# GloryyrolG/MHEntropy

Hardware: AMD Instinct MI355X
Metric: hypotheses/sec (BxK) fwd+loss, 256x256 (higher is better)
Workload: dtype bf16; 1 GPU; c2: MHEnt.get_loss forward+loss, resnet50 encoder (train-mode BN), 12-coupling RealNVP h=512, MANO joints, B=256/GPU, K=64, 256x256; images_per_gpu=256, hypotheses_per_image=64, global_batch=256, launch=hip-graph replay, base_noise=drawn on the device inside the step (Philox4x32-10, mhe_randn_f32), timing=one window of 452 steps, bracketed by barrier + synchronize, ranks=1, rccl_ranks=0

## Files before the change

### mhentropy_amd/csrc/conv_stream.hip

```cpp
#include "conv_shared.h"

namespace mhe { namespace conv {

constexpr int ST_PIX = 64;

template <int KT, int ST_BN, bool BNLOAD, bool DG = false>
__global__ __launch_bounds__(256, (ST_BN * KT + 2 * ST_PIX * KT) * 128 + ST_PIX * ST_BN * 2 <= 80 * 1024 ? 2 : 1)
void conv1x1_stream_kernel(const Params p, int nchunks, int ntiles_n) {
    using T = u16;
    constexpr int NTH = 256, CPR = ST_BN * 2 / 16;
    constexpr int NTW = ST_BN / 64, NJ = ST_PIX * CPR / NTH;
    constexpr int SWM = CPR < 16 ? CPR - 1 : 15;
    __shared__ uint4 Wl[ST_BN * 8 * KT];
    __shared__ uint4 Al[2][ST_PIX * 8 * KT];
    __shared__ uint4 Ol[ST_PIX * CPR > NTH * 4 ? ST_PIX * CPR : NTH * 4];
    const int tid = threadIdx.x, wave = tid >> 6, lane = tid & 63, q = lane >> 4, l15 = lane & 15;
    const int nt_id = blockIdx.x % ntiles_n, wg = blockIdx.x / ntiles_n, nwg = gridDim.x / ntiles_n;
    const int n0 = nt_id * ST_BN;
    const int s = tid & 7, rbase = tid >> 3;
    const T *xg = reinterpret_cast<const T *>(p.x);
    const T *wg_ = reinterpret_cast<const T *>(p.w);
    T *yg = reinterpret_cast<T *>(p.y);

#pragma unroll
    for (int kt = 0; kt < KT; ++kt)
#pragma unroll
        for (int j = 0; j < ST_BN / 32; ++j) {
            const int r = rbase + 32 * j, n = n0 + r;
            const uint4 v = n < p.Cout ? *reinterpret_cast<const uint4 *>(wg_ + (size_t)n * p.Kpad + kt * 64 + s * 8) : make_uint4(0, 0, 0, 0);
            Wl[kt * ST_BN * 8 + swz(r, s)] = v;
        }
    float sc[KT][8], sh[KT][8];
    if constexpr (BNLOAD) {
#pragma unroll
        for (int kt = 0; kt < KT; ++kt)
#pragma unroll
            for (int i = 0; i < 8; ++i) { sc[kt][i] = p.in_scale[kt * 64 + s * 8 + i]; sh[kt][i] = p.in_shift[kt * 64 + s * 8 + i]; }
    }
    uint4 ra[KT][2];
    auto load_chunk = [&](int c) {
#pragma unroll
        for (int kt = 0; kt < KT; ++kt)
#pragma unroll
            for (int j = 0; j < 2; ++j) {
                const long m = (long)c * ST_PIX + rbase + 32 * j;
                ra[kt][j] = (c < nchunks && m < p.M) ? *reinterpret_cast<const uint4 *>(xg + (size_t)m * p.Cin + kt * 64 + s * 8) : make_uint4(0, 0, 0, 0);
            }
    };
    auto store_chunk = [&](int buf, int c) {
#pragma unroll
        for (int kt = 0; kt < KT; ++kt)
#pragma unroll
            for (int j = 0; j < 2; ++j) {
                uint4 v = ra[kt][j];
                if constexpr (BNLOAD) {
                    const long m = (long)c * ST_PIX + rbase + 32 * j;
                    if (m < p.M) {
                        float f[8];
                        Chunk<T>::unpack(v, f);
#pragma unroll
                        for (int i = 0; i < 8; ++i) {
                            f[i] = fmaf(f[i], sc[kt][i], sh[kt][i]);
                            if (p.relu_in) f[i] = fmaxf(f[i], 0.f);
                        }
                        v = Chunk<T>::pack(f);
                    }
                }
                Al[buf][kt * ST_PIX * 8 + swz(rbase + 32 * j, s)] = v;
            }
    };
    const bool st_on = !DG && p.stats != nullptr;
    float ss1[8], ss2[8];
#pragma unroll
    for (int i = 0; i < 8; ++i) ss1[i] = ss2[i] = 0.f;
    const int ccol = n0 + (tid % CPR) * 8;
    const T *mk = reinterpret_cast<const T *>(p.mask), *rg = reinterpret_cast<const T *>(p.residual);
    const T *y0g = reinterpret_cast<const T *>(p.bn_y[0]), *y1g = reinterpret_cast<const T *>(p.bn_y[1]);
    const unsigned char *mkb = DG ? p.mask_bits : nullptr;
    const bool y0sum = DG && y0g != nullptr && y0g == mk, y1sum = DG && y1g != nullptr && y1g == mk;
    float bs1[DG ? 2 : 1][8], bs2[DG ? 2 : 1][8], bmu[DG ? 2 : 1][8], biv[DG ? 2 : 1][8];
    if constexpr (DG) {
#pragma unroll
        for (int u = 0; u < 2; ++u)
#pragma unroll
            for (int i = 0; i < 8; ++i) {
                const bool ok = p.bn_y[u] != nullptr && ccol + i < p.Cout;
                bs1[u][i] = bs2[u][i] = 0.f;
                bmu[u][i] = ok ? p.bn_mi[u][ccol + i] : 0.f;
                biv[u][i] = ok ? p.bn_mi[u][p.Cout + ccol + i] : 0.f;
            }
    }

    uint4 gm[DG ? 4 : 1], rr[DG ? 4 : 1], ya[DG ? 4 : 1], yb[DG ? 4 : 1];
    unsigned gmb[DG ? 4 : 1];
    size_t off[DG ? 4 : 1];
    bool okr[DG ? 4 : 1];
    auto dg_load = [&](int j0, int c) __attribute__((always_inline)) {
        if constexpr (DG) {
#pragma unroll
            for (int g = 0; g < 4; ++g) {
                const int id = tid + NTH * (j0 + g), row = id / CPR;
                const long m = (long)c * ST_PIX + row;
                okr[g] = m < p.M && ccol < p.Cout;
                const long mc = okr[g] ? m : 0;
                off[g] = (size_t)mc * p.Cout + ccol;
                if (mkb) gmb[g] = mkb[(size_t)mc * (p.Cout / 8) + (ccol >> 3)];
                else gm[g] = *reinterpret_cast<const uint4 *>(mk + off[g]);
                rr[g] = make_uint4(0u, 0u, 0u, 0u);
                if (rg) {
                    if (p.res_s2) {
                        const long hr = res_half_row(p, mc);
                        if (hr >= 0) rr[g] = *reinterpret_cast<const uint4 *>(rg + (size_t)hr * p.Cout + ccol);
                    } else rr[g] = *reinterpret_cast<const uint4 *>(rg + off[g]);
                }
                if (y0g && !y0sum) ya[g] = *reinterpret_cast<const uint4 *>(y0g + off[g]);
                if (y1g && !y1sum) yb[g] = *reinterpret_cast<const uint4 *>(y1g + off[g]);
            }
        }
    };
    load_chunk(wg);
    int it = 0;
    for (int c = wg; c < nchunks; c += nwg, ++it) {
        const int buf = it & 1;
        store_chunk(buf, c);
        load_chunk(c + nwg);
        if constexpr (ST_BN <= 128) dg_load(0, c);
        __syncthreads();
        v4f acc[NTW][4];
#pragma unroll
        for (int a = 0; a < NTW; ++a)
#pragma unroll
            for (int b = 0; b < 4; ++b) acc[a][b] = v4f{0.f, 0.f, 0.f, 0.f};
#pragma unroll
        for (int kt = 0; kt < KT; ++kt)
#pragma unroll
            for (int kk = 0; kk < 2; ++kk) {
                uint4 fa[4], fb[NTW];
#pragma unroll
                for (int mt = 0; mt < 4; ++mt) fa[mt] = Al[buf][kt * ST_PIX * 8 + swz(mt * 16 + l15, kk * 4 + q)];
#pragma unroll
                for (int nt = 0; nt < NTW; ++nt) fb[nt] = Wl[kt * ST_BN * 8 + swz(wave * (ST_BN / 4) + nt * 16 + l15, kk * 4 + q)];
#pragma unroll
                for (int nt = 0; nt < NTW; ++nt)
#pragma unroll
                    for (int mt = 0; mt < 4; ++mt)
                        acc[nt][mt] = __builtin_amdgcn_mfma_f32_16x16x32_bf16(
                            __builtin_bit_cast(__attribute__((ext_vector_type(8))) __bf16, fb[nt]),
                            __builtin_bit_cast(__attribute__((ext_vector_type(8))) __bf16, fa[mt]), acc[nt][mt], 0, 0, 0);
            }
        {
            unsigned char *ot = reinterpret_cast<unsigned char *>(Ol);
#pragma unroll
            for (int nt = 0; nt < NTW; ++nt)
#pragma unroll
                for (int mt = 0; mt < 4; ++mt) {
                    const int row = mt * 16 + l15, boff = (wave * (ST_BN / 4) + nt * 16 + 4 * q) * 2;
                    const int chunk = (boff >> 4) ^ (row & SWM);
                    const v4f v = acc[nt][mt];
                    uint2 o;
                    o.x = (unsigned)f32_to_bf16(v[0]) | ((unsigned)f32_to_bf16(v[1]) << 16);
                    o.y = (unsigned)f32_to_bf16(v[2]) | ((unsigned)f32_to_bf16(v[3]) << 16);
                    *reinterpret_cast<uint2 *>(ot + ((size_t)row * CPR + chunk) * 16 + (boff & 15)) = o;
                }
        }
        __syncthreads();
        {
            const unsigned char *ot = reinterpret_cast<const unsigned char *>(Ol);
            if constexpr (DG) {
#pragma unroll 1
                for (int j0 = 0; j0 < NJ; j0 += 4) {
                    if (j0 || ST_BN > 128) dg_load(j0, c);
                    uint4 raw[4];
#pragma unroll
                    for (int g = 0; g < 4; ++g) {
                        const int id = tid + NTH * (j0 + g), row = id / CPR, cc = id % CPR;
                        raw[g] = *reinterpret_cast<const uint4 *>(ot + ((size_t)row * CPR + (cc ^ (row & SWM))) * 16);
                    }
#pragma unroll
                    for (int g = 0; g < 4; ++g) {
                        if (!okr[g]) continue;
                        float v[8], t[8];
                        Chunk<T>::unpack(raw[g], v);
                        if (rg) {
                            Chunk<T>::unpack(rr[g], t);
#pragma unroll
                            for (int i = 0; i < 8; ++i) v[i] += t[i];
                        }
                        if (mkb) {
#pragma unroll
                            for (int i = 0; i < 8; ++i) v[i] = ((gmb[g] >> i) & 1u) ? v[i] : 0.f;
                        } else {
                            Chunk<T>::unpack(gm[g], t);
#pragma unroll
                            for (int i = 0; i < 8; ++i) v[i] = t[i] > 0.f ? v[i] : 0.f;
                        }
                        if (y0sum) {
#pragma unroll
                            for (int i = 0; i < 8; ++i) bs1[0][i] += v[i];
                        } else if (y0g) {
                            Chunk<T>::unpack(ya[g], t);
#pragma unroll
                            for (int i = 0; i < 8; ++i) { bs1[0][i] += v[i]; bs2[0][i] = fmaf(v[i], (t[i] - bmu[0][i]) * biv[0][i], bs2[0][i]); }
                        }
                        if (y1sum) {
#pragma unroll
                            for (int i = 0; i < 8; ++i) bs1[1][i] += v[i];
                        } else if (y1g) {
                            Chunk<T>::unpack(yb[g], t);
#pragma unroll
                            for (int i = 0; i < 8; ++i) { bs1[1][i] += v[i]; bs2[1][i] = fmaf(v[i], (t[i] - bmu[1][i]) * biv[1][i], bs2[1][i]); }
                        }
                        *reinterpret_cast<uint4 *>(yg + off[g]) = Chunk<T>::pack(v);
                    }
                }
                continue;
            }
            uint4 raw[NJ];
#pragma unroll
            for (int j = 0; j < NJ; ++j) {
                const int id = tid + NTH * j, row = id / CPR, cc = id % CPR;
                raw[j] = *reinterpret_cast<const uint4 *>(ot + ((size_t)row * CPR + (cc ^ (row & SWM))) * 16);
            }
#pragma unroll
            for (int j = 0; j < NJ; ++j) {
                const int id = tid + NTH * j, row = id / CPR, cc = id % CPR;
                const long m = (long)c * ST_PIX + row;
                const int n = n0 + cc * 8;
                if (m < p.M && n < p.Cout) {
                    if (st_on) {
                        float f[8];
                        Chunk<T>::unpack(raw[j], f);
#pragma unroll
                        for (int i = 0; i < 8; ++i) { ss1[i] += f[i]; ss2[i] = fmaf(f[i], f[i], ss2[i]); }
                    }
                    if (yg) *reinterpret_cast<uint4 *>(yg + (size_t)m * p.Cout + n) = raw[j];
                }
            }
        }
    }
    if constexpr (DG) {
        float *red = reinterpret_cast<float *>(Ol);
#pragma unroll
        for (int u = 0; u < 2; ++u) {
            if (!p.bn_y[u]) continue;
            __syncthreads();
#pragma unroll
            for (int i = 0; i < 8; ++i) { red[tid * 16 + i] = bs1[u][i]; red[tid * 16 + 8 + i] = bs2[u][i]; }
            __syncthreads();
            const int cch = tid / 8, e = tid % 8, n = n0 + tid;
            float a = 0.f, b = 0.f;
            if (tid < ST_BN)
                for (int k = 0; k < NTH / CPR; ++k) { a += red[(cch + CPR * k) * 16 + e]; b += red[(cch + CPR * k) * 16 + 8 + e]; }
            if (tid < ST_BN && n < p.Cout) {
                fx::add(p.bn_stats[u], wg % NSH, 0, p.Cout, n, a);
                fx::add(p.bn_stats[u], wg % NSH, 1, p.Cout, n, b);
            }
        }
    }
    if (st_on) {
        float *red = reinterpret_cast<float *>(Ol);
        __syncthreads();
#pragma unroll
        for (int i = 0; i < 8; ++i) { red[tid * 16 + i] = ss1[i]; red[tid * 16 + 8 + i] = ss2[i]; }
        __syncthreads();
        const int cch = tid / 8, e = tid % 8, n = n0 + tid;
        float a = 0.f, b = 0.f;
        if (tid < ST_BN)
            for (int k = 0; k < NTH / CPR; ++k) { a += red[(cch + CPR * k) * 16 + e]; b += red[(cch + CPR * k) * 16 + 8 + e]; }
        if (tid < ST_BN && n < p.Cout) {
            const int shard = wg % NSH;
            fx::add(p.stats, shard, 0, p.Cout, n, a);
            fx::add(p.stats, shard, 1, p.Cout, n, b);
        }
    }
}

__device__ __forceinline__ int swz3(int row, int slot) { return row * 8 + (slot ^ (((row >> 1) & 3) << 1)); }

template <bool BNLOAD, bool DG>
__global__ __launch_bounds__(512) void conv3x3_c64_stream_kernel(const Params p) {
    using T = u16;
    constexpr int NTH = 512, NT2 = 256, CPR = 8, WPX = 64, RROW = (WPX + 2) * 8;
    __shared__ uint4 Wl[9 * 64 * 8];
    __shared__ uint4 Rl[6][RROW];
    __shared__ uint4 Ol[2][1024];
    const int tid = threadIdx.x, wave = tid >> 6, lane = tid & 63, q = lane >> 4, l15 = lane & 15;
    const bool mult = wave < 4;
    const int t2 = tid & (NT2 - 1);
    const int s = t2 & 7, pbase = t2 >> 3;
    const int wrow = (wave >> 1) & 1, wpx = (wave & 1) * 32;
    const T *xg = reinterpret_cast<const T *>(p.x);
    const T *wg_ = reinterpret_cast<const T *>(p.w);
    T *yg = reinterpret_cast<T *>(p.y);
    const int H = p.H;
    const int npair = (H + 1) / 2 + 1;
    const int nimg = (p.B - (int)blockIdx.x + (int)gridDim.x - 1) / (int)gridDim.x;
    const int NT = nimg * npair;
    for (int i = tid; i < 9 * 64 * 8; i += NTH) {
        const int sl = i & 7, co = (i >> 3) & 63, tap = i >> 9;
        Wl[tap * 512 + swz3(co, sl)] = *reinterpret_cast<const uint4 *>(wg_ + (size_t)co * p.Kpad + tap * 64 + sl * 8);
    }
    if (tid < 6 * 16) {
        const int b = tid >> 4, sl = tid & 7, px = (tid & 8) ? WPX + 1 : 0;
        Rl[b][swz3(px, sl)] = make_uint4(0, 0, 0, 0);
    }
    const bool st_on = !DG && p.stats != nullptr;
    float ss1[8], ss2[8];
#pragma unroll
    for (int i = 0; i < 8; ++i) ss1[i] = ss2[i] = 0.f;
    const int ccol = (t2 % CPR) * 8;
    float bs1[DG ? 2 : 1][8], bs2[DG ? 2 : 1][8];
#pragma unroll
    for (int u = 0; u < (DG ? 2 : 1); ++u)
#pragma unroll
        for (int i = 0; i < 8; ++i) bs1[u][i] = bs2[u][i] = 0.f;

    if (mult) {
        int ck = 0, sp = 2, sc_ = 0;
        for (int t = 0; t <= NT; ++t) {
            __syncthreads();
            if (t < NT && ck >= 1) {
                v4f acc[4][2];
#pragma unroll
                for (int a = 0; a < 4; ++a) { acc[a][0] = v4f{0.f, 0.f, 0.f, 0.f}; acc[a][1] = v4f{0.f, 0.f, 0.f, 0.f}; }
                uint4 fa[2][2], fb[2][4];
                auto frag = [&](int i, int bi) __attribute__((always_inline)) {
                    const int kh = i / 6, kw = (i / 2) % 3, kk = i & 1;
                    const int d = wrow + kh;
                    const uint4 *row = Rl[(d < 2 ? sp : sc_) * 2 + (d & 1)];
#pragma unroll
                    for (int mt = 0; mt < 2; ++mt) fa[bi][mt] = row[swz3(wpx + mt * 16 + l15 + kw, kk * 4 + q)];
#pragma unroll
                    for (int nt = 0; nt < 4; ++nt) fb[bi][nt] = Wl[(kh * 3 + kw) * 512 + swz3(nt * 16 + l15, kk * 4 + q)];
                };
                frag(0, 0);
#pragma unroll
                for (int i = 0; i < 18; ++i) {
                    if (i + 1 < 18) frag(i + 1, (i + 1) & 1);
                    __builtin_amdgcn_sched_barrier(0);
#pragma unroll
                    for (int nt = 0; nt < 4; ++nt)
#pragma unroll
                        for (int mt = 0; mt < 2; ++mt)
                            acc[nt][mt] = __builtin_amdgcn_mfma_f32_16x16x32_bf16(
                                __builtin_bit_cast(__attribute__((ext_vector_type(8))) __bf16, fb[i & 1][nt]),
                                __builtin_bit_cast(__attribute__((ext_vector_type(8))) __bf16, fa[i & 1][mt]), acc[nt][mt], 0, 0, 0);
                    __builtin_amdgcn_sched_barrier(0);
                }
                unsigned char *ot = reinterpret_cast<unsigned char *>(Ol[t & 1]);
#pragma unroll
                for (int nt = 0; nt < 4; ++nt)
#pragma unroll
                    for (int mt = 0; mt < 2; ++mt) {
                        const int row = wrow * WPX + wpx + mt * 16 + l15, boff = (nt * 16 + 4 * q) * 2;
                        const int chunk = (boff >> 4) ^ (row & 7);
                        const v4f v = acc[nt][mt];
                        uint2 o;
                        o.x = (unsigned)f32_to_bf16(v[0]) | ((unsigned)f32_to_bf16(v[1]) << 16);
                        o.y = (unsigned)f32_to_bf16(v[2]) | ((unsigned)f32_to_bf16(v[3]) << 16);
                        *reinterpret_cast<uint2 *>(ot + ((size_t)row * CPR + chunk) * 16 + (boff & 15)) = o;
                    }
            }
            sp = sc_;
            sc_ = sc_ == 2 ? 0 : sc_ + 1;
            if (++ck == npair) ck = 0;
        }
    } else {
        float sc[8], sh[8];
        if constexpr (BNLOAD) {
#pragma unroll
            for (int i = 0; i < 8; ++i) { sc[i] = p.in_scale[s * 8 + i]; sh[i] = p.in_shift[s * 8 + i]; }
        }
        const T *mk = reinterpret_cast<const T *>(p.mask), *rg = reinterpret_cast<const T *>(p.residual);
        const T *y0g = reinterpret_cast<const T *>(p.bn_y[0]), *y1g = reinterpret_cast<const T *>(p.bn_y[1]);
        float bmu[DG ? 2 : 1][8], biv[DG ? 2 : 1][8];
        if constexpr (DG) {
#pragma unroll
            for (int u = 0; u < 2; ++u)
#pragma unroll
                for (int i = 0; i < 8; ++i) {
                    const bool ok = p.bn_y[u] != nullptr;
                    bmu[u][i] = ok ? p.bn_mi[u][ccol + i] : 0.f;
                    biv[u][i] = ok ? p.bn_mi[u][64 + ccol + i] : 0.f;
                }
        }
        uint4 ra[2][2][2];
        auto load_pair = [&](int img, int k, auto SET) __attribute__((always_inline)) {
            constexpr int set = decltype(SET)::value;
            const size_t b = (size_t)blockIdx.x + (size_t)img * gridDim.x;
#pragma unroll
            for (int e = 0; e < 2; ++e)
#pragma unroll
                for (int j = 0; j < 2; ++j)
                    ra[set][e][j] = (unsigned)(2 * k - 1 + e) < (unsigned)H
                                        ? *reinterpret_cast<const uint4 *>(xg + ((b * H + 2 * k - 1 + e) * WPX + pbase + 32 * j) * 64 + s * 8)
                                        : make_uint4(0, 0, 0, 0);
        };
        auto store_pair = [&](int k, int slot, auto SET) __attribute__((always_inline)) {
            constexpr int set = decltype(SET)::value;
#pragma unroll
            for (int e = 0; e < 2; ++e)
#pragma unroll
                for (int j = 0; j < 2; ++j) {
                    uint4 v = ra[set][e][j];
                    if constexpr (BNLOAD) {
                        if ((unsigned)(2 * k - 1 + e) < (unsigned)H) {
                            float f[8];
                            Chunk<T>::unpack(v, f);
#pragma unroll
                            for (int i = 0; i < 8; ++i) {
                                f[i] = fmaf(f[i], sc[i], sh[i]);
                                if (p.relu_in) f[i] = fmaxf(f[i], 0.f);
                            }
                            v = Chunk<T>::pack(f);
                        }
                    }
                    Rl[slot * 2 + e][swz3(pbase + 32 * j + 1, s)] = v;
                }
        };
        uint4 gm[DG ? 4 : 1], rr[DG ? 4 : 1], ya[DG ? 4 : 1], yb[DG ? 4 : 1];
        auto dg_load = [&](int img, int k) __attribute__((always_inline)) {
            if constexpr (DG) {
                const int y = 2 * (k - 1);
                const size_t m0 = (((size_t)blockIdx.x + (size_t)img * gridDim.x) * H + y) * WPX;
                const int nrows = (y + 1 < H ? 2 : 1) * WPX;
#pragma unroll
                for (int j = 0; j < 4; ++j) {
                    const int row = (t2 + NT2 * j) / CPR;
                    const size_t off = (m0 + (row < nrows ? row : 0)) * 64 + ccol;
                    gm[j] = *reinterpret_cast<const uint4 *>(mk + off);
                    rr[j] = rg ? *reinterpret_cast<const uint4 *>(rg + off) : make_uint4(0, 0, 0, 0);
                    if (y0g) ya[j] = *reinterpret_cast<const uint4 *>(y0g + off);
                    if (y1g) yb[j] = *reinterpret_cast<const uint4 *>(y1g + off);
                }
            }
        };
        auto epilogue = [&](int img, int k, int par) __attribute__((always_inline)) {
            const unsigned char *ot = reinterpret_cast<const unsigned char *>(Ol[par]);
            const int y = 2 * (k - 1);
            const size_t m0 = (((size_t)blockIdx.x + (size_t)img * gridDim.x) * H + y) * WPX;
            const int nrows = (y + 1 < H ? 2 : 1) * WPX;
            uint4 raw[4];
#pragma unroll
            for (int j = 0; j < 4; ++j) {
                const int id = t2 + NT2 * j, row = id / CPR, cc = id % CPR;
                raw[j] = *reinterpret_cast<const uint4 *>(ot + ((size_t)row * CPR + (cc ^ (row & 7))) * 16);
            }
#pragma unroll
            for (int j = 0; j < 4; ++j) {
                const int id = t2 + NT2 * j, row = id / CPR;
                if (row >= nrows) continue;
                const size_t off = (m0 + row) * 64 + ccol;
                if constexpr (DG) {
                    float v[8], t[8];
                    Chunk<T>::unpack(raw[j], v);
                    if (rg) {
                        Chunk<T>::unpack(rr[j], t);
#pragma unroll
                        for (int i = 0; i < 8; ++i) v[i] += t[i];
                    }
                    Chunk<T>::unpack(gm[j], t);
#pragma unroll
                    for (int i = 0; i < 8; ++i) v[i] = t[i] > 0.f ? v[i] : 0.f;
                    if (y0g) {
                        Chunk<T>::unpack(ya[j], t);
#pragma unroll
                        for (int i = 0; i < 8; ++i) { bs1[0][i] += v[i]; bs2[0][i] = fmaf(v[i], (t[i] - bmu[0][i]) * biv[0][i], bs2[0][i]); }
                    }
                    if (y1g) {
                        Chunk<T>::unpack(yb[j], t);
#pragma unroll
                        for (int i = 0; i < 8; ++i) { bs1[1][i] += v[i]; bs2[1][i] = fmaf(v[i], (t[i] - bmu[1][i]) * biv[1][i], bs2[1][i]); }
                    }
                    *reinterpret_cast<uint4 *>(yg + off) = Chunk<T>::pack(v);
                } else {
                    if (st_on) {
                        float f[8];
                        Chunk<T>::unpack(raw[j], f);
#pragma unroll
                        for (int i = 0; i < 8; ++i) { ss1[i] += f[i]; ss2[i] = fmaf(f[i], f[i], ss2[i]); }
                    }
                    *reinterpret_cast<uint4 *>(yg + off) = raw[j];
                }
            }
        };
        using S0 = std::integral_constant<int, 0>;
        using S1 = std::integral_constant<int, 1>;
        int li = 0, lk = 0;
        auto next_load = [&](auto SET) __attribute__((always_inline)) {
            if (li < nimg) load_pair(li, lk, SET);
            if (++lk == npair) { lk = 0; ++li; }
        };
        next_load(S0{});
        store_pair(0, 0, S0{});
        next_load(S1{});
        next_load(S0{});
        int wk = 1, ws = 1;
        int ci = 0, ck = 0, pi = 0, pk = 0;
        auto tick = [&](int t, auto SET) __attribute__((always_inline)) {
            __syncthreads();
            if (t + 1 < NT) store_pair(wk, ws, SET);
            if (++wk == npair) wk = 0;
            ws = ws == 2 ? 0 : ws + 1;
            if (t >= 1 && pk >= 1) epilogue(pi, pk, (t - 1) & 1);
            next_load(SET);
            if (t < NT && ck >= 1) dg_load(ci, ck);
            pi = ci; pk = ck;
            if (++ck == npair) { ck = 0; ++ci; }
        };
        for (int t = 0; t <= NT; t += 2) {
            tick(t, S1{});
            if (t + 1 <= NT) tick(t + 1, S0{});
        }
    }
    float *red = reinterpret_cast<float *>(Ol[0]);
    auto fold = [&](const float *a8, const float *b8, fx::acc_t *dst) __attribute__((always_inline)) {
        __syncthreads();
        if (!mult) {
#pragma unroll
            for (int i = 0; i < 8; ++i) { red[t2 * 16 + i] = a8[i]; red[t2 * 16 + 8 + i] = b8[i]; }
        }
        __syncthreads();
        if (!mult && t2 < 64) {
            const int cch = t2 / 8, e = t2 % 8;
            float a = 0.f, b = 0.f;
            for (int k = 0; k < NT2 / CPR; ++k) { a += red[(cch + CPR * k) * 16 + e]; b += red[(cch + CPR * k) * 16 + 8 + e]; }
            fx::add(dst, (int)(blockIdx.x % NSH), 0, 64, t2, a);
            fx::add(dst, (int)(blockIdx.x % NSH), 1, 64, t2, b);
        }
    };
    if constexpr (DG) {
#pragma unroll
        for (int u = 0; u < 2; ++u)
            if (p.bn_y[u]) fold(bs1[u], bs2[u], p.bn_stats[u]);
    } else if (st_on) fold(ss1, ss2, p.stats);
}

bool stream3_supports(const Params &p) {
    if (!(p.KH == 3 && p.KW == 3 && p.stride == 1 && p.pad == 1 && p.Cin == 64 && p.Cout == 64 && p.W == 64 && p.Kpad == 576 && p.B >= 128 &&
          p.H >= 16 && !p.x2 && !p.out_scale && !p.out_shift && !p.relu_out && !p.y32 && !p.os2 && !p.a_out && !p.res_s2))
        return false;
    if (p.mask) return !p.in_scale && !p.stats;
    return !p.residual;
}

int launch_stream3(const Params &p, hipStream_t s) {
    const dim3 grid((unsigned)(p.B < 256 ? p.B : 256)), block(512);
    if (p.mask) hipLaunchKernelGGL((conv3x3_c64_stream_kernel<false, true>), grid, block, 0, s, p);
    else if (p.in_scale) hipLaunchKernelGGL((conv3x3_c64_stream_kernel<true, false>), grid, block, 0, s, p);
    else hipLaunchKernelGGL((conv3x3_c64_stream_kernel<false, false>), grid, block, 0, s, p);
    return check_launch("conv3x3_c64_stream_kernel");
}

static int stream_bn(const Params &p) { return p.Cin == 64 ? (p.Cout == 64 && !p.mask ? 64 : 256) : (p.Cin == 128 && !p.mask ? 256 : 128); }

bool stream_supports(const Params &p) {
    if (!(p.KH == 1 && p.KW == 1 && p.stride == 1 && p.pad == 0 && (p.Cin == 64 || p.Cin == 128 || p.Cin == 256) && p.Kpad == p.Cin &&
          !p.x2 && !p.out_scale && !p.out_shift && !p.relu_out && !p.y32 && !p.os2 && !p.a_out && (p.M >= 64 * 1024 || (p.stats_only && !p.mask))))
        return false;
    if (p.Cout % stream_bn(p)) return false;
    if (p.Cin == 256 && !p.mask) return false;
    if (p.mask) return !p.in_scale && !p.stats;
    return !p.residual;
}

template <int KT, int NB>
static void launch_stream_t(const Params &p, hipStream_t s, dim3 grid, int nchunks, int ntn) {
    const dim3 block(256);
    if constexpr (NB == 64) {
        if (p.in_scale) hipLaunchKernelGGL((conv1x1_stream_kernel<KT, NB, true>), grid, block, 0, s, p, nchunks, ntn);
        else hipLaunchKernelGGL((conv1x1_stream_kernel<KT, NB, false>), grid, block, 0, s, p, nchunks, ntn);
    } else if (p.mask) hipLaunchKernelGGL((conv1x1_stream_kernel<KT, NB, false, true>), grid, block, 0, s, p, nchunks, ntn);
    else if constexpr (KT <= 2) {
        if (p.in_scale) hipLaunchKernelGGL((conv1x1_stream_kernel<KT, NB, true>), grid, block, 0, s, p, nchunks, ntn);
        else hipLaunchKernelGGL((conv1x1_stream_kernel<KT, NB, false>), grid, block, 0, s, p, nchunks, ntn);
    } else hipLaunchKernelGGL((conv1x1_stream_kernel<KT, NB, false>), grid, block, 0, s, p, nchunks, ntn);
}

int launch_stream(const Params &p, hipStream_t s) {
    const int nb = stream_bn(p);
    const int nchunks = (p.M + ST_PIX - 1) / ST_PIX, ntn = p.Cout / nb;
    const int per_cu = nb == 64 ? 4 : (p.Cin == 256 || (p.Cin == 128 && nb == 256)) ? 1 : 2;
    int nwg = 256 * per_cu / ntn;
    if (nwg < 1) nwg = 1;
    if (nwg > nchunks) nwg = nchunks;
    const dim3 grid((unsigned)(nwg * ntn));
    if (p.Cin == 64 && nb == 64) launch_stream_t<1, 64>(p, s, grid, nchunks, ntn);
    else if (p.Cin == 64) launch_stream_t<1, 256>(p, s, grid, nchunks, ntn);
    else if (p.Cin == 128 && nb == 256) launch_stream_t<2, 256>(p, s, grid, nchunks, ntn);
    else if (p.Cin == 128) launch_stream_t<2, 128>(p, s, grid, nchunks, ntn);
    else launch_stream_t<4, 128>(p, s, grid, nchunks, ntn);
    return check_launch("conv1x1_stream_kernel");
}

}}
```

### mhentropy_amd/ops.py

```python
import ctypes as C
import os

import numpy as np
import torch

from . import _lib
from ._lib import ConvDesc, check

F32, BF16 = 0, 1
FLOW_FORWARD, FLOW_INVERSE = 0, 1

TIMING = False
TIMING_DG = False
KERNEL_TIMES = []


def _stream():
    return C.c_void_p(torch.cuda.current_stream().cuda_stream)


def _ptr(t):
    return C.c_void_p(0 if t is None else t.data_ptr())


def _chk(t, dtype, name, shape=None):
    if not isinstance(t, torch.Tensor) or not t.is_cuda:
        raise _lib.MheError(f"{name}: expected a CUDA/HIP tensor (the hot path has no CPU fallback)")
    if t.dtype != dtype:
        raise _lib.MheError(f"{name}: expected {dtype}, got {t.dtype}")
    if not t.is_contiguous():
        raise _lib.MheError(f"{name}: must be contiguous")
    if shape is not None and tuple(t.shape) != tuple(shape):
        raise _lib.MheError(f"{name}: expected shape {tuple(shape)}, got {tuple(t.shape)}")
    return t


def launch(entry, *args):
    conv = []
    for i, a in enumerate(args):
        if a is None or isinstance(a, torch.Tensor):
            if a is not None and not a.is_cuda:
                raise _lib.MheError(f"{entry}: argument {i} is a {a.device.type} tensor, every tensor operand must be device memory (the hot path has no CPU fallback)")
            a = _ptr(a)
        conv.append(a)
    check(getattr(_lib.lib(), entry)(*conv, _stream()), entry)


class _Timed:
    def __init__(self, what):
        self.what = what if TIMING else None

    def __enter__(self):
        if self.what is not None:
            self.rec = self.what()
            self.ev0, self.ev1 = torch.cuda.Event(enable_timing=True), torch.cuda.Event(enable_timing=True)
            self.ev0.record()
        return self

    def __exit__(self, exc_type, *exc):
        if self.what is not None and exc_type is None:
            self.ev1.record()
            name, flops, nbytes = self.rec
            KERNEL_TIMES.append((name, flops, self.ev0, self.ev1, nbytes))
        return False


def _bn_consumers(bn, n, dt, shape, Cn, prefix, only_one=None):
    bn = list(bn or [])
    if only_one and len(bn) > 1:
        raise ValueError(only_one)
    flat = []
    for by, bmi, bst in (bn + [(None, None, None)] * n)[:n]:
        if by is not None:
            _chk(by, dt, prefix + ".bn_y", shape); _chk(bmi, torch.float32, prefix + ".bn_mean_invstd", (2, Cn))
            _chk_stats(bst, prefix + ".bn_stats", Cn)
        flat += [by, bmi, bst]
    return flat


def _grow_only_workspace():
    live, retired = {}, []

    def get(device, need):
        ws = live.get(device)
        if ws is None or ws.numel() < need:
            if ws is not None:
                retired.append(ws)
            ws = live[device] = torch.empty(need, device=device, dtype=torch.float32)
        return ws
    return get


def stat_shards():
    return _lib.lib().mhe_conv_stat_shards()


STAT_DTYPE = torch.int64


def stat_shape(C):
    return (2, stat_shards(), 2, C)


def stat_unit(C, device):
    return torch.zeros(stat_shape(C), device=device, dtype=STAT_DTYPE)


def stat_totals(st):
    t = st.sum(1)
    return t[0].double() * 2.0 ** -16 + t[1].double() * 2.0 ** -56


def stat_from_float(t):
    d = t.double() * 2.0 ** 16
    hi = torch.round(d)
    lo = torch.round((d - hi) * 2.0 ** 40)
    return torch.stack([hi.to(torch.int64), lo.to(torch.int64)]).contiguous()


def _chk_stats(t, name, C):
    _chk(t, STAT_DTYPE, name, stat_shape(C))


_TILES = {0: "128, 64, 2, 2", 1: "128, 128, 2, 2", 2: "256, 256, 2, 4", 3: "256, 128, 4, 2", 4: "256, 64, 4, 2"}


def _conv_kernel_name(d, dt, mode):
    bke = 32 if dt == torch.float32 else 64
    tile = _lib.lib().mhe_conv_tile_mode(C.byref(d), mode)
    mode = 0 if mode == 3 else mode
    if tile == 11:
        return "mhe::conv::conv_wide_kernel<%s, %s>" % ("128, 4" if d.Cin == 256 else "64, 8", "true" if mode == 1 else "false")
    if tile == 10:
        return "mhe::conv::conv_tail_kernel<false>"
    if tile == 9:
        return "mhe::conv::conv3x3_c64_stream_kernel<%s, false>" % ("true" if mode == 1 else "false")
    if tile == 8:
        return "mhe::conv::conv1x1_stream_kernel<%d, %d, %s, false>" % (d.Cin // 64, 64 if (d.Cin == 64 and d.Cout == 64) else 256 if d.Cin <= 128 else 128, "true" if mode == 1 else "false")
    if tile == 13:
        return "mhe::conv::conv_p8_kernel<false, %s, 0, 1>" % ("false" if d.KH == 1 and d.KW == 1 and d.pad == 0 else "true")
    if tile == 7:
        return "mhe::conv::conv_p8_kernel<false, %s, 0, 2>" % ("false" if d.KH == 1 and d.KW == 1 and d.pad == 0 else "true")
    return "mhe::conv::conv_kernel<%s, %s, %s, %d, false>" % ("float" if dt == torch.float32 else "unsigned short",
                                                             _TILES[tile],
                                                             "true" if d.Cin % bke == 0 else "false", mode)


def dtype_code(dt):
    return F32 if dt == torch.float32 else BF16


def conv_tile_choice(B, H, W, Cin, Cout, k, stride, pad, dt, mode=0):
    d = ConvDesc(B, H, W, Cin, Cout, k, k, stride, pad, dtype_code(dt), int(mode == 1), 0, 0, 0)
    return _lib.lib().mhe_conv_tile_mode(C.byref(d), mode)


def linear(x, w, bias=None, relu=False, out=None, want_bf16=False):
    M, K = x.shape
    N = w.shape[0]
    _chk(x, torch.float32, "linear.x"); _chk(w, torch.float32, "linear.w", (N, K))
    if bias is not None:
        _chk(bias, torch.float32, "linear.bias", (N,))
    y = out if out is not None else torch.empty(M, N, device=x.device, dtype=torch.float32)
    _chk(y, torch.float32, "linear.out", (M, N))
    if want_bf16:
        if M <= 256 and K % 64 == 0 and N % 4 == 0:
            yb = torch.empty(M, N, device=x.device, dtype=torch.bfloat16)
            launch("mhe_linear_f32_bf16copy", x, w, bias, y, yb, M, N, K, int(relu))
            return y, yb
        launch("mhe_linear_f32", x, w, bias, y, M, N, K, int(relu))
        return y, None
    launch("mhe_linear_f32", x, w, bias, y, M, N, K, int(relu))
    return y


_RNG_STATE = {}


def rng_state(device, seed=None):
    device = torch.device(device)
    if device.type == "cuda" and device.index is None:
        device = torch.device("cuda", torch.cuda.current_device())
    st = _RNG_STATE.get(device)
    if st is None:
        s = torch.initial_seed() if seed is None else int(seed)
        st = _RNG_STATE[device] = torch.tensor([s & 0x7FFFFFFFFFFFFFFF, 0, 0], dtype=torch.int64, device=device)
    elif seed is not None:
        st.copy_(torch.tensor([int(seed) & 0x7FFFFFFFFFFFFFFF, 0, 0], dtype=torch.int64))
    return st


def rng_get_state(device):
    return rng_state(device).cpu().clone()


def rng_set_state(device, words):
    st = rng_state(device)
    st.copy_(torch.as_tensor(words, dtype=torch.int64).reshape(3))
    return st


def randn(rows, cols, device, scale=1.0, state=None):
    out = torch.empty(rows, cols, device=device, dtype=torch.float32)
    st = state if state is not None else rng_state(out.device)
    launch("mhe_randn_f32", out, out.numel(), st, float(scale))
    return out


def dropout_(x, p, bits=None, state=None):
    if x.dtype not in (torch.float32, torch.bfloat16) or not x.is_cuda or not x.is_contiguous() or x.numel() % 8:
        raise _lib.MheError("dropout_: contiguous f32 / bf16 device tensor with a multiple of 8 elements expected")
    draw = bits is None
    if draw:
        bits = torch.empty(x.numel() // 8, device=x.device, dtype=torch.uint8)
        st = state if state is not None else rng_state(x.device)
    else:
        _chk(bits, torch.uint8, "dropout.bits", (x.numel() // 8,))
        st = None
    launch("mhe_dropout", x, dtype_code(x.dtype), bits, x.numel(), float(p), st, int(draw))
    return bits


def dropout_mask(bits, shape, p):
    m = ((bits.view(-1, 1).int() >> torch.arange(8, device=bits.device, dtype=torch.int32)) & 1).float().reshape(shape)
    return m / (1.0 - p)


def reparam(mn, l2, eps=None, sigmoid_act=False, deterministic=False):
    _chk(mn, torch.float32, "reparam.mn"); _chk(l2, torch.float32, "reparam.l2", mn.shape)
    if eps is not None:
        _chk(eps, torch.float32, "reparam.eps", mn.shape)
    sd, z = torch.empty_like(mn), torch.empty_like(mn)
    launch("mhe_reparam_f32", mn, l2, eps, sd, z, mn.numel(), int(sigmoid_act), int(deterministic or eps is None))
    return sd, z


def flow_pack_net(w0, w1, w2):
    hidden, dim = w0.shape
    L = _lib.lib()
    n = L.mhe_flow_packed_floats_per_net(dim, hidden)
    if n == 0:
        raise _lib.MheError(f"flow_pack_net: unsupported geometry dim={dim} hidden={hidden}")
    out = np.empty(n, np.float32)
    w0, w1, w2 = (np.ascontiguousarray(a, np.float32) for a in (w0, w1, w2))
    check(L.mhe_flow_pack_net_host(w0.ctypes.data_as(C.c_void_p), w1.ctypes.data_as(C.c_void_p),
                                   w2.ctypes.data_as(C.c_void_p), dim, hidden, out.ctypes.data_as(C.c_void_p)),
          "mhe_flow_pack_net_host")
    return out


def flow_pack_net_bf16(w0, w1, w2):
    hidden, dim = w0.shape
    L = _lib.lib()
    n = L.mhe_flow_packed_bytes_per_net_bf16(dim, hidden)
    if n == 0:
        raise _lib.MheError(f"flow_pack_net_bf16: unsupported geometry dim={dim} hidden={hidden}")
    out = np.empty(n // 2, np.uint16)
    w0, w1, w2 = (np.ascontiguousarray(a, np.float32) for a in (w0, w1, w2))
    check(L.mhe_flow_pack_net_bf16_host(w0.ctypes.data_as(C.c_void_p), w1.ctypes.data_as(C.c_void_p),
                                        w2.ctypes.data_as(C.c_void_p), dim, hidden, out.ctypes.data_as(C.c_void_p)),
          "mhe_flow_pack_net_bf16_host")
    return out


def flow_couplings(x_in, cond, wstream, bias2, mask, B, hidden, direction, want_log_prob=True):
    R, dim = x_in.shape
    ncoup = mask.shape[0]
    _chk(x_in, torch.float32, "flow.in")
    _chk(cond, torch.float32, "flow.cond", (B, 2 * ncoup, 2, hidden))
    bf16 = wstream.dtype != torch.float32
    _chk(wstream, wstream.dtype, "flow.wstream"); _chk(bias2, torch.float32, "flow.bias2", (2 * ncoup, 64 if bf16 else dim))
    _chk(mask, torch.float32, "flow.mask", (ncoup, dim))
    out = torch.empty_like(x_in)
    sum_s = torch.empty(R, device=x_in.device, dtype=torch.float32)
    logp = torch.empty(R, device=x_in.device, dtype=torch.float32) if want_log_prob else None
    launch("mhe_flow_couplings_bf16" if bf16 else "mhe_flow_couplings_f32", x_in, out, cond, wstream, bias2, mask, sum_s, logp, R, B, dim, hidden, ncoup,
           direction)
    return out, sum_s, logp


def flow_couplings_emit(x_in, cond, wstream, bias2, mask, B, hidden, direction, h1, h2, o):
    R, dim = x_in.shape
    ncoup = mask.shape[0]
    _chk(x_in, torch.float32, "flow.in"); _chk(cond, torch.float32, "flow.cond", (B, 2 * ncoup, 2, hidden))
    _chk(wstream, wstream.dtype, "flow.wstream"); _chk(bias2, torch.float32, "flow.bias2", (2 * ncoup, 64))
    _chk(mask, torch.float32, "flow.mask", (ncoup, dim))
    _chk(h1, torch.bfloat16, "flow.h1", (2 * ncoup, R, hidden)); _chk(h2, torch.bfloat16, "flow.h2", (2 * ncoup, R, hidden))
    _chk(o, torch.float32, "flow.o", (2 * ncoup, R, 64))
    out = torch.empty_like(x_in)
    sum_s = torch.empty(R, device=x_in.device, dtype=torch.float32)
    logp = torch.empty(R, device=x_in.device, dtype=torch.float32)
    launch("mhe_flow_couplings_bf16_emit", x_in, out, cond, wstream, bias2, mask, sum_s, logp, h1, h2, o, R, B, dim, hidden, ncoup, direction)
    return out, sum_s, logp


def flow_couplings_frag_supported(R, B, dim, hidden, ncoup):
    return bool(_lib.lib().mhe_flow_couplings_frag_supported(R, B, dim, hidden, ncoup))


def flow_frag_pack(w0, w1, w2):
    h, dim = w0.shape
    fill = -1 if not w0.is_floating_point() else 0
    w0p = torch.full((h, 64), fill, dtype=w0.dtype, device=w0.device); w0p[:, :dim] = w0
    w2p = torch.full((64, h), fill, dtype=w2.dtype, device=w2.device); w2p[:dim] = w2
    return mfma_fragment_major(w1), mfma_fragment_major(w0p), mfma_fragment_major(w2p)


def flow_couplings_frag(x_in, cond, w0F, w1F, w2F, w_net_stride, bias2, mask, B, hidden, direction, want_log_prob=True, emit=None, sign_bits=None):
    R, dim = x_in.shape
    ncoup = mask.shape[0]
    _chk(x_in, torch.float32, "flow.in"); _chk(cond, torch.float32, "flow.cond", (B, 2 * ncoup, 2, hidden))
    _chk(bias2, torch.float32, "flow.bias2", (2 * ncoup, 64)); _chk(mask, torch.float32, "flow.mask", (ncoup, dim))
    for t, nm in ((w0F, "w0F"), (w1F, "w1F"), (w2F, "w2F")):
        _chk(t, torch.bfloat16, "flow." + nm)
    h1 = h2 = o = None
    if emit is not None:
        h1, h2, o = emit
        _chk(h1, torch.bfloat16, "flow.h1", (2 * ncoup, R, hidden)); _chk(h2, torch.bfloat16, "flow.h2", (2 * ncoup, R, hidden))
        _chk(o, torch.float32, "flow.o", (2 * ncoup, R, 64))
    if sign_bits is not None:
        _chk(sign_bits, torch.int32, "flow.sign_bits", (2 * ncoup, R // 64, 2, 8, 64, 2))
    out = torch.empty_like(x_in)
    sum_s = torch.empty(R, device=x_in.device, dtype=torch.float32)
    logp = torch.empty(R, device=x_in.device, dtype=torch.float32) if want_log_prob else None
    launch("mhe_flow_couplings_frag_bf16", x_in, out, cond, 4 * ncoup * hidden, w0F, w1F, w2F, int(w_net_stride), bias2, mask, sum_s, logp, h1, h2, o, sign_bits, R,
           B, dim, hidden, ncoup, direction)
    return out, sum_s, logp


MODS_UV, MODS_XYZ = 1, 2


def mods_bits(mods):
    if mods is None:
        return MODS_UV
    names = [mods] if isinstance(mods, str) else list(mods)
    bits = 0
    for m in names:
        if m not in ("uv", "xyz"):
            raise NotImplementedError(f"mods={names!r}: only the 'uv' and 'xyz' likelihoods are built (hand/network.py:620-643)")
        bits |= MODS_UV if m == "uv" else MODS_XYZ
    if not bits or len(names) != len(set(names)):
        raise NotImplementedError(f"mods={names!r}: expected ['uv'], ['xyz'] or ['xyz', 'uv']")
    return bits


def _chamfer_target(chamfer, B, who):
    if not isinstance(chamfer, (tuple, list)) or len(chamfer) != 4:
        raise ValueError(f"{who}: chamfer must be (scale, root, obj, count)")
    scale, root, obj, count = chamfer
    if not isinstance(obj, torch.Tensor) or obj.dim() != 3:
        raise _lib.MheError(f"{who}.obj: expected a [B,VO,3] tensor")
    VO = obj.shape[1]
    _chk(scale, torch.float32, f"{who}.scale", (B,)); _chk(root, torch.float32, f"{who}.root", (B, 3)); _chk(obj, torch.float32, f"{who}.obj", (B, VO, 3))
    if count is not None:
        _chk(count, torch.int32, f"{who}.count", (B,))
    return VO


def mano_joints(th45, det, tables, crop_uv=None, vis=None, laplace_b=0.03, th45_alpha=50.0, inv_norm=False,
                image_size=256.0, want=("z", "xyz", "uv", "terms", "log_p", "norms"), pose3d=None, mods=None, laplace_b_3d=0.03,
                chamfer=None):
    R, B = th45.shape[0], det.shape[0]
    dev = th45.device
    _chk(th45, torch.float32, "mano.th45", (R, 45)); _chk(det, torch.float32, "mano.det", (B, 16))
    _chk(tables, torch.float32, "mano.tables")
    if crop_uv is not None:
        _chk(crop_uv, torch.float32, "mano.crop_uv", (B, 42))
    if vis is not None:
        _chk(vis, torch.float32, "mano.vis", (B, 21))
    if pose3d is not None:
        _chk(pose3d, torch.float32, "mano.pose3d", (B, 63))
    bits = None if mods is None else (int(mods) if isinstance(mods, int) else mods_bits(mods))
    if chamfer is not None:
        VO = _chamfer_target(chamfer, B, "mano.chamfer")
        if vis is None:
            raise ValueError("mano_joints(chamfer=...): vis is required")
        if "verts" in want or "mesh_mm" in want:
            raise ValueError("mano_joints: the mesh outputs come from the uv-only pass (mods=None, chamfer=None)")
        bits = MODS_UV if bits is None else bits
        shapes = {"z": (R, 61), "xyz": (R, 63), "uv": (R, 42), "terms": (R, 5), "log_p": (R,), "norms": (R, 2), "joints_mm": (R, 63)}
        o = {k: (torch.empty(shapes[k], device=dev, dtype=torch.float32) if k in want else None) for k in shapes}
        o["chamfer"] = torch.empty(R, device=dev, dtype=torch.float32)
        launch("mhe_mano_joints_chamfer_f32", th45, det, crop_uv, vis, pose3d, tables, *chamfer, o["z"], o["xyz"], o["uv"], o["terms"], o["log_p"],
               o["norms"], o["joints_mm"], o["chamfer"], R, B, VO, bits, float(laplace_b), float(laplace_b_3d), float(th45_alpha), int(inv_norm),
               float(image_size))
        return o
    shapes = {"z": (R, 61), "xyz": (R, 63), "uv": (R, 42), "terms": (R, 4 if bits is None else 5), "log_p": (R,), "norms": (R, 2),
              "joints_mm": (R, 63)}
    o = {k: (torch.empty(shapes[k], device=dev, dtype=torch.float32) if k in want else None) for k in shapes}
    if bits is not None:
        if "verts" in want or "mesh_mm" in want:
            raise ValueError("mano_joints: the mesh outputs come from the uv-only pass (mods=None)")
        launch("mhe_mano_joints_mods_f32", th45, det, crop_uv, vis, pose3d, tables, o["z"], o["xyz"], o["uv"], o["terms"], o["log_p"], o["norms"], o["joints_mm"], R,
               B, bits, float(laplace_b), float(laplace_b_3d), float(th45_alpha), int(inv_norm), float(image_size))
        return o
    if "verts" in want or "mesh_mm" in want:
        if "verts" in want and "mesh_mm" in want:
            raise ValueError("mano_joints: 'verts' or 'mesh_mm', one mesh per call")
        key = "verts" if "verts" in want else "mesh_mm"
        o[key] = torch.empty(R, 778, 3, device=dev, dtype=torch.float32)
        ws = torch.empty(_lib.lib().mhe_mano_verts_workspace_floats(R), device=dev, dtype=torch.float32)
        launch("mhe_mano_decode_f32", th45, det, crop_uv, vis, tables, o["z"], o["xyz"], o["uv"], o["terms"], o["log_p"], o["norms"], o["joints_mm"], o[key], ws, R,
               B, float(laplace_b), float(th45_alpha), int(inv_norm), float(image_size), int(key == "mesh_mm"))
        return o
    launch("mhe_mano_joints_f32", th45, det, crop_uv, vis, tables, o["z"], o["xyz"], o["uv"], o["terms"], o["log_p"], o["norms"], o["joints_mm"], R, B,
           float(laplace_b), float(th45_alpha), int(inv_norm), float(image_size))
    return o


def mano_joints_bwd(th45, det, tables, crop_uv, vis, g_log_p, N, laplace_b=0.03, th45_alpha=50.0, pose3d=None, mods=None,
                    laplace_b_3d=0.03, chamfer=None, chamfer_w=0.0):
    R, B = th45.shape[0], det.shape[0]
    _chk(th45, torch.float32, "mano_bwd.th45", (R, 45)); _chk(det, torch.float32, "mano_bwd.det", (B, 16))
    if crop_uv is not None or mods is None:
        _chk(crop_uv, torch.float32, "mano_bwd.crop_uv", (B, 42))
    _chk(vis, torch.float32, "mano_bwd.vis", (B, 21))
    if pose3d is not None:
        _chk(pose3d, torch.float32, "mano_bwd.pose3d", (B, 63))
    _chk(g_log_p, torch.float32, "mano_bwd.g_log_p", (B,))
    g_th45 = torch.empty(R, 45, device=th45.device, dtype=torch.float32)
    g_rows = torch.empty(R, 16, device=th45.device, dtype=torch.float32)
    if chamfer is not None:
        VO = _chamfer_target(chamfer, B, "mano_bwd.chamfer")
        bits = MODS_UV if mods is None else (int(mods) if isinstance(mods, int) else mods_bits(mods))
        launch("mhe_mano_joints_chamfer_bwd_f32", th45, det, crop_uv, vis, pose3d, tables, *chamfer, g_log_p, g_th45, g_rows, R, B, VO, bits,
               float(laplace_b), float(laplace_b_3d), float(th45_alpha), 1.0 / N, float(chamfer_w))
    elif mods is None:
        launch("mhe_mano_joints_bwd_f32", th45, det, crop_uv, vis, tables, g_log_p, g_th45, g_rows, R, B, float(laplace_b), float(th45_alpha), 1.0 / N)
    else:
        bits = int(mods) if isinstance(mods, int) else mods_bits(mods)
        launch("mhe_mano_joints_mods_bwd_f32", th45, det, crop_uv, vis, pose3d, tables, g_log_p, g_th45, g_rows, R, B, bits, float(laplace_b), float(laplace_b_3d),
               float(th45_alpha), 1.0 / N)
    return g_th45, sum_over_hypotheses(g_rows, N, B)


def sum_over_hypotheses(rows, N, B, out=None, accumulate=False, out_stride=0):
    Cc = rows.shape[1]
    _chk(rows, torch.float32, "sum_over_hypotheses.rows", (N * B, Cc))
# ... 1238 lines not shown
```

Measured before the change: 2.548 million hypotheses/s.

## Split 3x3 c64 stream conv into three warp roles for BN-input path

Adds a 768-thread variant of the 3x3 64-channel streaming conv for the BN-folded input case. Waves 0-3 still do the MMA, waves 4-7 now only load and stage inputs, and a new set of waves 8-11 runs the epilogue and statistics fold. The aim is to take epilogue stores off the loader's critical path so loads and stores overlap better. The cost is a larger block with more registers and barrier participants, which may lower occupancy or add sync overhead.

Measured after the change: 2.575 million hypotheses/s (median of 6 runs). +1.1%, better.

```diff
diff --git a/mhentropy_amd/csrc/conv_stream.hip b/mhentropy_amd/csrc/conv_stream.hip
--- a/mhentropy_amd/csrc/conv_stream.hip
+++ b/mhentropy_amd/csrc/conv_stream.hip
@@ -277,15 +277,17 @@
 
 __device__ __forceinline__ int swz3(int row, int slot) { return row * 8 + (slot ^ (((row >> 1) & 3) << 1)); }
 
-template <bool BNLOAD, bool DG>
-__global__ __launch_bounds__(512) void conv3x3_c64_stream_kernel(const Params p) {
+template <bool BNLOAD, bool DG, int ROLES>
+__device__ __forceinline__ void conv3x3_c64_stream_body(const Params &p) {
+    static_assert(ROLES == 2 || (ROLES == 3 && !DG), "the data-gradient form keeps its two roles");
     using T = u16;
-    constexpr int NTH = 512, NT2 = 256, CPR = 8, WPX = 64, RROW = (WPX + 2) * 8;
+    constexpr int NTH = 256 * ROLES, NT2 = 256, CPR = 8, WPX = 64, RROW = (WPX + 2) * 8;
     __shared__ uint4 Wl[9 * 64 * 8];
     __shared__ uint4 Rl[6][RROW];
     __shared__ uint4 Ol[2][1024];
     const int tid = threadIdx.x, wave = tid >> 6, lane = tid & 63, q = lane >> 4, l15 = lane & 15;
     const bool mult = wave < 4;
+    const bool storer = !mult && (ROLES == 2 || wave >= 8);
     const int t2 = tid & (NT2 - 1);
     const int s = t2 & 7, pbase = t2 >> 3;
     const int wrow = (wave >> 1) & 1, wpx = (wave & 1) * 32;
@@ -368,8 +370,10 @@
     } else {
         float sc[8], sh[8];
         if constexpr (BNLOAD) {
-#pragma unroll
-            for (int i = 0; i < 8; ++i) { sc[i] = p.in_scale[s * 8 + i]; sh[i] = p.in_shift[s * 8 + i]; }
+            if (ROLES == 2 || wave < 8) {
+#pragma unroll
+                for (int i = 0; i < 8; ++i) { sc[i] = p.in_scale[s * 8 + i]; sh[i] = p.in_shift[s * 8 + i]; }
+            }
         }
         const T *mk = reinterpret_cast<const T *>(p.mask), *rg = reinterpret_cast<const T *>(p.residual);
         const T *y0g = reinterpret_cast<const T *>(p.bn_y[0]), *y1g = reinterpret_cast<const T *>(p.bn_y[1]);
@@ -491,37 +495,50 @@
             if (li < nimg) load_pair(li, lk, SET);
             if (++lk == npair) { lk = 0; ++li; }
         };
-        next_load(S0{});
-        store_pair(0, 0, S0{});
-        next_load(S1{});
-        next_load(S0{});
-        int wk = 1, ws = 1;
         int ci = 0, ck = 0, pi = 0, pk = 0;
-        auto tick = [&](int t, auto SET) __attribute__((always_inline)) {
-            __syncthreads();
-            if (t + 1 < NT) store_pair(wk, ws, SET);
-            if (++wk == npair) wk = 0;
-            ws = ws == 2 ? 0 : ws + 1;
-            if (t >= 1 && pk >= 1) epilogue(pi, pk, (t - 1) & 1);
-            next_load(SET);
-            if (t < NT && ck >= 1) dg_load(ci, ck);
-            pi = ci; pk = ck;
-            if (++ck == npair) { ck = 0; ++ci; }
-        };
-        for (int t = 0; t <= NT; t += 2) {
-            tick(t, S1{});
-            if (t + 1 <= NT) tick(t + 1, S0{});
+        if (ROLES == 2 || wave < 8) {
+            next_load(S0{});
+            store_pair(0, 0, S0{});
+            next_load(S1{});
+            next_load(S0{});
+            int wk = 1, ws = 1;
+            auto tick = [&](int t, auto SET) __attribute__((always_inline)) {
+                __syncthreads();
+                if (t + 1 < NT) store_pair(wk, ws, SET);
+                if (++wk == npair) wk = 0;
+                ws = ws == 2 ? 0 : ws + 1;
+                if constexpr (ROLES == 2) {
+                    if (t >= 1 && pk >= 1) epilogue(pi, pk, (t - 1) & 1);
+                }
+                next_load(SET);
+                if constexpr (ROLES == 2) {
+                    if (t < NT && ck >= 1) dg_load(ci, ck);
+                    pi = ci; pk = ck;
+                    if (++ck == npair) { ck = 0; ++ci; }
+                }
+            };
+            for (int t = 0; t <= NT; t += 2) {
+                tick(t, S1{});
+                if (t + 1 <= NT) tick(t + 1, S0{});
+            }
+        } else {
+            for (int t = 0; t <= NT; ++t) {
+                __syncthreads();
+                if (t >= 1 && pk >= 1) epilogue(pi, pk, (t - 1) & 1);
+                pi = ci; pk = ck;
+                if (++ck == npair) { ck = 0; ++ci; }
+            }
         }
     }
     float *red = reinterpret_cast<float *>(Ol[0]);
     auto fold = [&](const float *a8, const float *b8, fx::acc_t *dst) __attribute__((always_inline)) {
         __syncthreads();
-        if (!mult) {
+        if (storer) {
 #pragma unroll
             for (int i = 0; i < 8; ++i) { red[t2 * 16 + i] = a8[i]; red[t2 * 16 + 8 + i] = b8[i]; }
         }
         __syncthreads();
-        if (!mult && t2 < 64) {
+        if (storer && t2 < 64) {
             const int cch = t2 / 8, e = t2 % 8;
             float a = 0.f, b = 0.f;
             for (int k = 0; k < NT2 / CPR; ++k) { a += red[(cch + CPR * k) * 16 + e]; b += red[(cch + CPR * k) * 16 + 8 + e]; }
@@ -535,6 +552,11 @@
             if (p.bn_y[u]) fold(bs1[u], bs2[u], p.bn_stats[u]);
     } else if (st_on) fold(ss1, ss2, p.stats);
 }
+
+template <bool BNLOAD, bool DG>
+__global__ __launch_bounds__(512) void conv3x3_c64_stream_kernel(const Params p) { conv3x3_c64_stream_body<BNLOAD, DG, 2>(p); }
+template <bool BNLOAD>
+__global__ __launch_bounds__(768) void conv3x3_c64_roles3_kernel(const Params p) { conv3x3_c64_stream_body<BNLOAD, false, 3>(p); }
 
 bool stream3_supports(const Params &p) {
     if (!(p.KH == 3 && p.KW == 3 && p.stride == 1 && p.pad == 1 && p.Cin == 64 && p.Cout == 64 && p.W == 64 && p.Kpad == 576 && p.B >= 128 &&
@@ -545,10 +567,10 @@
 }
 
 int launch_stream3(const Params &p, hipStream_t s) {
-    const dim3 grid((unsigned)(p.B < 256 ? p.B : 256)), block(512);
-    if (p.mask) hipLaunchKernelGGL((conv3x3_c64_stream_kernel<false, true>), grid, block, 0, s, p);
-    else if (p.in_scale) hipLaunchKernelGGL((conv3x3_c64_stream_kernel<true, false>), grid, block, 0, s, p);
-    else hipLaunchKernelGGL((conv3x3_c64_stream_kernel<false, false>), grid, block, 0, s, p);
+    const dim3 grid((unsigned)(p.B < 256 ? p.B : 256));
+    if (p.mask) hipLaunchKernelGGL((conv3x3_c64_stream_kernel<false, true>), grid, dim3(512), 0, s, p);
+    else if (p.in_scale) hipLaunchKernelGGL((conv3x3_c64_roles3_kernel<true>), grid, dim3(768), 0, s, p);
+    else hipLaunchKernelGGL((conv3x3_c64_stream_kernel<false, false>), grid, dim3(512), 0, s, p);
     return check_launch("conv3x3_c64_stream_kernel");
 }
 
diff --git a/mhentropy_amd/ops.py b/mhentropy_amd/ops.py
--- a/mhentropy_amd/ops.py
+++ b/mhentropy_amd/ops.py
@@ -134,7 +134,7 @@
     if tile == 10:
         return "mhe::conv::conv_tail_kernel<false>"
     if tile == 9:
-        return "mhe::conv::conv3x3_c64_stream_kernel<%s, false>" % ("true" if mode == 1 else "false")
+        return "mhe::conv::conv3x3_c64_roles3_kernel<true>" if mode == 1 else "mhe::conv::conv3x3_c64_stream_kernel<false, false>"
     if tile == 8:
         return "mhe::conv::conv1x1_stream_kernel<%d, %d, %s, false>" % (d.Cin // 64, 64 if (d.Cin == 64 and d.Cout == 64) else 256 if d.Cin <= 128 else 128, "true" if mode == 1 else "false")
     if tile == 13:
```
